# hzheng40/irbfn

Measured on AMD Instinct MI355X. Metric: RBF-net evals/s (B queries x N centres), forward, higher is better.
Workload: dtype f32 (distances and Phi x W on f16 MFMA: exact fixed-point heads + float tails, hi/lo operand pairs; f32 accumulate)

## Files before the change

irbfn_amd/csrc/pack_all.hip:

```cpp
#include <hip/hip_runtime.h>
#include <math.h>
#include <stdint.h>

#include "rbf_forward_gram.h"

namespace irbfn {

constexpr int kPackBlock = 256;
constexpr int kStatsCentres = 1024;
constexpr int kStatsVals = 18;
constexpr int kGramLdsMax = gram_chunk_bytes(8);

struct PackArgs {
  const float* __restrict__ centers;
  const float* __restrict__ log_sigs;
  const float* __restrict__ kernel;
  const float* __restrict__ bias;
  float* __restrict__ rec;
  float* __restrict__ bias_out;
  float* __restrict__ sig2;
  float* __restrict__ recm;
  float* __restrict__ oscale;
  unsigned char* __restrict__ f16_img;
  unsigned char* __restrict__ gram_img;
  GramHdr* __restrict__ hdr;
  float* __restrict__ part;
// ... 245 lines not shown
__device__ __forceinline__ void gram_image_body(const PackArgs& a, int c, unsigned char* simg, GramHdr& hs, float* tot) {
  const int tid = threadIdx.x;
  if (tid < kStatsVals) {
    float m = a.part[tid];
    for (int b = 1; b < a.nbS; ++b) m = fmaxf(m, a.part[(size_t)b * kStatsVals + tid]);
    tot[tid] = m;
  }
  __syncthreads();
  if (tid == 0) {
    hs = gram_header(tot, a.D, a.bclass, a.gscale);
    if (c == 0) *a.hdr = hs;
  }
  __syncthreads();
  const GramHdr h = hs;
  const int NT = a.NT, D = a.D;
  const int CB = gram_chunk_bytes(NT);
  unsigned char* p = simg;
  for (int it = tid; it < kF16Chunk * 16; it += kPackBlock) {
    const int part = it >> 5, kk = it & 31;
    const int reg = c / a.cpr, kr = (c - reg * a.cpr) * kF16Chunk + kk;
    const int n = reg * a.KR + kr;
    const bool real = kr < a.KR;
    const int ct = kk >> 4, row = kk & 15;
    _Float16* head = reinterpret_cast<_Float16*>(p + ct * 512);
    auto put_head = [&](int s, double v, int T) { head[((s >> 2) * 16 + row) * 4 + (s & 3)] = (_Float16)(float)(v * gram_pow2(T - gram_ax(T))); };
    auto put_tail = [&](int s, double v, int T) {
      const int half = s >> 5, g = (s >> 3) & 3, j = s & 7;
      _Float16* tail = reinterpret_cast<_Float16*>(p + kGramHeadBytes + (ct * 2 + half) * 1024);
      tail[(g * 16 + row) * 8 + j] = (_Float16)(float)(v * gram_pow2(T - gram_ax(T)));
    };
    double alpha = 0.0, beta = 0.0;
    if (h.ok) {
      const double s2 = real ? (double)expf(-2.0f * a.log_sigs[n]) : 1.0;
      gram_alpha_beta(a.bclass, s2, a.gscale, alpha, beta);
      if (!real) alpha = 0.0;
    }
    auto centre_value = [&](const GramSlot sl) -> double {
      if (!h.ok || sl.kind == 0) return 0.0;
      if (sl.kind == 1) {
        double nC[3] = {0.0, 0.0, 0.0};
        if (real && sl.dim < D) gram_parts_d(-2.0 * alpha * ((double)a.centers[(size_t)n * D + sl.dim] - (double)h.r[sl.dim]), h.ec, nC);
        return sl.q == 0 ? nC[0] : (sl.q == 1 ? nC[1] : nC[2]);
      }
      if (sl.kind == 2) {
// ... 6 lines not shown
        for (int i = 0; i < D && i < kGramDims; ++i) {
          const double cp = (double)a.centers[(size_t)n * D + i] - (double)h.r[i];
          c2 += alpha * cp * cp;
        }
      gram_parts_c2(c2, h.e2, n2);
      return sl.p == 0 ? n2[0] : (sl.p == 1 ? n2[1] : (sl.p == 2 ? n2[2] : n2[3]));
    };
    {
      const GramSlot sl = gram_head_slot(part);
      put_head(part, centre_value(sl), gram_T(h, sl));
    }
    for (int i = 0; i < 4; ++i) {
      const GramSlot sl = gram_tail_slot(4 * part + i);
      put_tail(4 * part + i, centre_value(sl), gram_T(h, sl));
    }
    const int g = row >> 2, j = ct * 4 + (row & 3);
    for (int wt = 0; wt < NT; ++wt) {
      _Float16* wh = reinterpret_cast<_Float16*>(p + kGramOpBytes + (size_t)wt * 2 * kF16WBytes);
      _Float16* wl = wh + kF16WBytes / 2;
      const int oo = part, o = wt * 16 + oo;
      float w = 0.0f;
      if (real && o < a.O) w = a.kernel[(size_t)(n % a.K) * a.O + o] / a.oscale[o];
      _Float16 hh, ll;
      split_static_f16(w, hh, ll);
      wh[(g * 16 + oo) * 8 + j] = hh;
      wl[(g * 16 + oo) * 8 + j] = ll;
    }
  }
  __syncthreads();
  uint4* dst = reinterpret_cast<uint4*>(a.gram_img + (size_t)c * CB);
// ... 78 lines not shown
```

irbfn_amd/csrc/rbf_forward_gram.h:

```cpp
#pragma once

#include "rbf_forward_f16_narrow.h"

namespace irbfn {

typedef _Float16 h4_t __attribute__((ext_vector_type(4)));

constexpr int kGramHeadBytes = 2 * 64 * 8;
constexpr int kGramTailBytes = 2 * 2 * 64 * 16;
constexpr int kGramOpBytes = kGramHeadBytes + kGramTailBytes;
constexpr int gram_chunk_bytes(int NT = 1) { return kGramOpBytes + NT * 2 * kF16WBytes; }
constexpr int kGramChunkBytes = gram_chunk_bytes(1);
constexpr int kGramDims = 8;
#ifndef IRBFN_GRAM_RING
#define IRBFN_GRAM_RING 5
#endif
constexpr int kGramRing = IRBFN_GRAM_RING;
#ifndef IRBFN_GRAM_WAVES
#define IRBFN_GRAM_WAVES 4
#endif

struct GramHdr {
  float r[8];
  int ex, ec, eq, ea, e2;
  int ok;
  float cabs, amax, cmax, c2max;
};
// ... 3 lines not shown
__host__ __device__ constexpr int gram_comb_q(int m) { return m == 0 ? 1 : (m == 1 ? 0 : (m == 2 ? 2 : (m == 3 ? 0 : 1))); }
__host__ __device__ constexpr GramSlot gram_head_slot(int s) {
  const int g = s >> 2, j = s & 3;
  return j < 2 ? GramSlot{1, 2 * g + j, 0, 0}
               : (j == 2 ? (g == 0 ? GramSlot{2, 0, 0, 0} : (g == 1 ? GramSlot{3, 0, 0, 0} : (g == 2 ? GramSlot{3, 0, 1, 0} : GramSlot{0, 0, 0, 0})))
                         : GramSlot{0, 0, 0, 0});
}
__host__ __device__ constexpr GramSlot gram_tail_slot(int s) {
  const int hf = s >> 5, g = (s >> 3) & 3, j = s & 7;
  const int m = hf * 3 + (j - 5);
  return j < 5 ? GramSlot{1, 2 * g + hf, gram_comb_p(j), gram_comb_q(j)}
               : (g == 0 ? (m < 5 ? GramSlot{2, 0, gram_comb_p(m), gram_comb_q(m)} : GramSlot{3, 0, 2, 0})
                         : (g == 1 && hf == 0 && j == 5 ? GramSlot{3, 0, 3, 0} : GramSlot{0, 0, 0, 0}));
}
static_assert(kGramDims == 8, "four lane groups x two coordinates");
__host__ __device__ inline int gram_T(const GramHdr& h, const GramSlot sl) {
  return sl.kind == 1 ? h.ex + h.ec - 11 * (sl.p + sl.q) : (sl.kind == 2 ? h.eq + h.ea - 11 * (sl.p + sl.q) : h.e2 - 11 * sl.p);
}
__host__ __device__ inline int gram_ax(int T) { return (T + 1) >> 1; }

template <int BC>
__host__ __device__ constexpr float gram_phi_scale() { return BC == BC_IMQ ? 128.0f : kPhiScale; }

#ifdef IRBFN_GRAM_STAMPS
__device__ unsigned long long g_gram_stamps[64];
#define IRBFN_GRAM_T() __builtin_amdgcn_s_memtime()
#define IRBFN_GRAM_PHASE(k)                                                                            \
  do {                                                                                                 \
    asm volatile("s_waitcnt vmcnt(0) lgkmcnt(0)" ::: "memory");                                        \
    if (blockIdx.x < 2 && threadIdx.x == 0) {                                                          \
// ... 75 lines not shown
                                                 float (&rv)[2]) {
#pragma unroll
  for (int c = 0; c < 2; ++c) rv[c] = hp->r[2 * g + c];
#pragma unroll
  for (int t = 0; t < 2; ++t)
#pragma unroll
    for (int c = 0; c < 2; ++c) {
      const int i = 2 * g + c;
      const bool in = i < DC && i < a.Dreal;
      const float v = a.x[qrow[t] * a.Dreal + (in ? i : 0)];
      xv[t][c] = in ? v : 0.0f;
    }
}

template <int DC>
__device__ __forceinline__ bool gram_query_operands(const F16Args& a, const GramHdr* hp, const float (&xin)[2][2], const float (&rin)[2],
                                                    int g, h4_t (&bhd)[2], h8_t (&btl)[2][2]) {
#pragma clang fp contract(off)
  static_assert(DC <= kGramDims, "eight coordinate slots");
  const int ex = hp->ex, ec = hp->ec, eq = hp->eq, ea = hp->ea, e2 = hp->e2;
  GramHdr hx;
  hx.ex = ex; hx.ec = ec; hx.eq = eq; hx.ea = ea; hx.e2 = e2;
  bool bad = hp->ok == 0;
  const float xinv = __builtin_ldexpf(1.0f, -ex), qinv = __builtin_ldexpf(1.0f, -eq);
  const float xlim = __builtin_ldexpf(1.0f, ex) * 0.999f, qlim = __builtin_ldexpf(1.0f, eq) * 0.999f;
  auto scale_of = [&](const GramSlot sl) -> float { return sl.kind == 0 ? 0.0f : __builtin_ldexpf(1.0f, gram_ax(gram_T(hx, sl))); };
  float rr[2];
#pragma unroll
  for (int c = 0; c < 2; ++c) {
    rr[c] = (2 * g + c < DC) ? -rin[c] : 0.0f;
  }
#pragma unroll
  for (int t = 0; t < 2; ++t) {
    float nx[2][3], nq[3];
    float qh = 0.0f, ql = 0.0f;
#pragma unroll
    for (int c = 0; c < 2; ++c) {
      const float xv = xin[t][c];
      const float sh = xv + rr[c];
      const float bb = sh - xv;
      const float sl = (xv - (sh - bb)) + (rr[c] - bb);
      bad = bad || !(__builtin_fabsf(sh) < xlim);
      gram_parts_f(sh, sl, xinv, nx[c]);
      const float ph = sh * sh;
      const float pl = __builtin_fmaf(sh, sh, -ph) + 2.0f * sh * sl;
      const float th = qh + ph;
      const float tb = th - qh;
      ql += ((qh - (th - tb)) + (ph - tb)) + pl;
      qh = th;
    }
#pragma unroll
    for (int off = 16; off <= 32; off *= 2) {
      const float oh = __shfl_xor(qh, off), ol = __shfl_xor(ql, off);
      const float th = qh + oh;
      const float tb = th - qh;
      ql = ((qh - (th - tb)) + (oh - tb)) + (ql + ol);
      qh = th;
    }
    bad = bad || !(qh < qlim);
    gram_parts_f(qh, ql, qinv, nq);
    {
      const float sc = scale_of(gram_head_slot(0));
      const float f2 = g == 0 ? nq[0] * scale_of(gram_head_slot(2))
                              : (g == 1 ? scale_of(gram_head_slot(4 + 2)) : (g == 2 ? scale_of(gram_head_slot(8 + 2)) : 0.0f));
      bhd[t][0] = (_Float16)(nx[0][0] * sc);
      bhd[t][1] = (_Float16)(nx[1][0] * sc);
      bhd[t][2] = (_Float16)f2;
      bhd[t][3] = (_Float16)0.0f;
    }
#pragma unroll
    for (int hf = 0; hf < 2; ++hf) {
#pragma unroll
      for (int j = 0; j < 5; ++j) {
        const GramSlot sl = gram_tail_slot(32 * hf + j);
        btl[t][hf][j] = (_Float16)(nx[hf][sl.p] * scale_of(sl));
      }
#pragma unroll
      for (int j = 5; j < 8; ++j) {
        const GramSlot s0 = gram_tail_slot(32 * hf + j), s1 = gram_tail_slot(32 * hf + 8 + j);
        const float v0 = s0.kind == 2 ? nq[s0.p] * scale_of(s0) : scale_of(s0);
        const float v1 = scale_of(s1);
        btl[t][hf][j] = (_Float16)(g == 0 ? v0 : (g == 1 ? v1 : 0.0f));
      }
    }
  }
  return bad;
}
template <int DC>
__device__ __forceinline__ bool gram_query_operands(const F16Args& a, const GramHdr* hp, const long (&qrow)[2], int g, h4_t (&bhd)[2],
                                                    h8_t (&btl)[2][2]) {
  float xv[2][2], rv[2];
  gram_query_loads<DC>(a, hp, qrow, g, xv, rv);
  return gram_query_operands<DC>(a, hp, xv, rv, g, bhd, btl);
}
static_assert(gram_head_slot(0).kind == 1 && gram_head_slot(4 * 3 + 1).dim == 7 && gram_head_slot(2).kind == 2 && gram_head_slot(6).kind == 3 &&
              gram_head_slot(10).kind == 3 && gram_head_slot(10).p == 1 && gram_head_slot(14).kind == 0 && gram_head_slot(3).kind == 0, "head slots");
static_assert(gram_tail_slot(32 + 8 * 2 + 4).kind == 1 && gram_tail_slot(32 + 8 * 2 + 4).dim == 5 && gram_tail_slot(5).kind == 2 &&
              gram_tail_slot(32 + 6).kind == 2 && gram_tail_slot(32 + 7).kind == 3 && gram_tail_slot(32 + 7).p == 2 && gram_tail_slot(8 + 5).kind == 3 &&
              gram_tail_slot(8 + 5).p == 3 && gram_tail_slot(8 + 6).kind == 0 && gram_tail_slot(16 + 5).kind == 0 && gram_tail_slot(32 + 8 + 5).kind == 0, "tail slots");

__device__ __forceinline__ void gram_heads(const h4_t (&a)[2], const h4_t (&b)[2], f4_t (&u)[2][2]) {
  asm("v_mfma_f32_16x16x16_f16 %0, %4, %6, 0\n v_mfma_f32_16x16x16_f16 %1, %5, %6, 0\n v_mfma_f32_16x16x16_f16 %2, %4, %7, 0\n "
      "v_mfma_f32_16x16x16_f16 %3, %5, %7, 0\n s_nop 4"
      : "=&v"(u[0][0]), "=&v"(u[0][1]), "=&v"(u[1][0]), "=&v"(u[1][1])
      : "v"(a[0]), "v"(a[1]), "v"(b[0]), "v"(b[1]));
}
__device__ __forceinline__ void gram_heads2(const h4_t& a, const h4_t (&b)[2], f4_t (&u)[2]) {
  asm("v_mfma_f32_16x16x16_f16 %0, %2, %3, 0\n v_mfma_f32_16x16x16_f16 %1, %2, %4, 0\n s_nop 4"
      : "=&v"(u[0]), "=&v"(u[1])
      : "v"(a), "v"(b[0]), "v"(b[1]));
}

__device__ __forceinline__ void gram_heads2c(const h4_t& a, const h4_t (&b)[2], const f4_t& c, f4_t (&u)[2]) {
  asm("v_mfma_f32_16x16x16_f16 %0, %2, %3, %5\n v_mfma_f32_16x16x16_f16 %1, %2, %4, %5\n s_nop 4"
      : "=&v"(u[0]), "=&v"(u[1])
      : "v"(a), "v"(b[0]), "v"(b[1]), "v"(c));
}

__device__ __forceinline__ void gram_distances_at(const unsigned char* l8, const unsigned char* l16, const h4_t (&bhd)[2],
                                                  const h8_t (&btl)[2][2], f4_t (&u)[2][2]) {
  h4_t ahd[2];
  h8_t atl[2][2];
#pragma unroll
  for (int ct = 0; ct < 2; ++ct) {
    ahd[ct] = *reinterpret_cast<const h4_t*>(l8 + ct * 512);
    atl[ct][0] = *reinterpret_cast<const h8_t*>(l16 + kGramHeadBytes + (ct * 2 + 0) * 1024);
    atl[ct][1] = *reinterpret_cast<const h8_t*>(l16 + kGramHeadBytes + (ct * 2 + 1) * 1024);
  }
  gram_heads(ahd, bhd, u);
#pragma unroll
  for (int hf = 0; hf < 2; ++hf)
#pragma unroll
    for (int t = 0; t < 2; ++t)
#pragma unroll
      for (int ct = 0; ct < 2; ++ct)
        u[t][ct] = __builtin_amdgcn_mfma_f32_16x16x32_f16(atl[ct][hf], btl[t][hf], u[t][ct], 0, 0, 0);
}
__device__ __forceinline__ void gram_distances(const unsigned char* buf, int lane, const h4_t (&bhd)[2], const h8_t (&btl)[2][2],
                                               f4_t (&u)[2][2]) {
  gram_distances_at(buf + lane * 8, buf + lane * 16, bhd, btl, u);
}

template <int DC, int BC, bool FINITE_R2 = false>
__device__ __forceinline__ void gram_valu_args(const F16Args& a, const long (&qrow)[2], int g, const float* recs, float (&t16)[16]) {
  constexpr int RF = f16_rf(DC);
#pragma unroll
  for (int t = 0; t < 2; ++t) {
    float xq[DC];
#pragma unroll
    for (int d = 0; d < DC; ++d) xq[d] = d < a.Dreal ? a.x[qrow[t] * a.Dreal + d] : 0.0f;
#pragma unroll
    for (int j = 0; j < 8; ++j) {
      const float* rp = recs + ((j >> 2) * 16 + 4 * g + (j & 3)) * RF;
      float r2 = 0.0f;
#pragma unroll
// ... 18 lines not shown
```

irbfn_amd/csrc/rbf_forward_gram.hip:

```cpp
#include <hip/hip_fp16.h>
#include <stdint.h>
#include <stdio.h>
#include <stdlib.h>

#include "rbf_forward_gram_body.h"

namespace irbfn {

template <int DC, int BC>
__global__ __launch_bounds__(1024, IRBFN_GRAM_WAVES) void rbf_fwd_f16gram(const GramArgs ga) {
  extern __shared__ __attribute__((aligned(16))) unsigned char lds[];
  gram_body<DC, BC, false>(ga, F16Roll{}, -1, lds);
}

template <int DC, int BC>
__global__ __launch_bounds__(1024, IRBFN_GRAM_WAVES) void rbf_tick_f16gram(const GramArgs ga, const F16Roll rl, const int mode) {
  extern __shared__ __attribute__((aligned(16))) unsigned char lds[];
  gram_body<DC, BC, true>(ga, rl, mode, lds);
}

static int gram_nt(const irbfn_net* net) { return (net->O + 15) / 16; }

bool gram_eligible(const irbfn_net* net) {
  return f16_eligible(net) && net->DC <= kGramDims;
}

size_t gram_image_bytes(const irbfn_net* net) {
  const int nchunks = (net->N + kF16Chunk - 1) / kF16Chunk;
  return (size_t)nchunks * gram_chunk_bytes(gram_nt(net));
}

size_t gram_header_bytes() { return sizeof(GramHdr); }

#ifdef IRBFN_GRAM_STAMPS
extern "C" int irbfn_debug_gram_stamps(unsigned long long* out64) {
  return (int)hipMemcpyFromSymbol(out64, HIP_SYMBOL(g_gram_stamps), sizeof(unsigned long long) * 64);
}
#endif

size_t gram_lds_bytes(int S, int QG, bool tick, bool gamma) {
  size_t ring = (size_t)S * kGramRing * kGramChunkBytes;
  if (gamma) ring += (size_t)S * QG * 128 * sizeof(float);
  else ring += (size_t)QG * 32 * sizeof(float);
  size_t red = (size_t)S * QG * 2 * 4 * 64 + (size_t)QG * 32;
// ... 31 lines not shown
```

irbfn_amd/csrc/rbf_forward_gram_body.h:

```cpp
#pragma once

#include "rbf_forward_gram.h"

namespace irbfn {

struct GramGamma {
  const float* __restrict__ gamma;
  int R, cpr;
};

template <int DC, int BC, bool ROLL, bool GAMMA = false>
__device__ __forceinline__ void gram_body(const GramArgs& ga, const F16Roll& rl, int mode, unsigned char* lds,
                                          [[maybe_unused]] const GramGamma gm = GramGamma{nullptr, 1, 1}) {
  static_assert(DC <= kGramDims, "eight coordinate slots");
  const F16Args& a = ga.f;
  constexpr int CBL = f16_chunk_bytes(DC);
  constexpr int CB = kGramChunkBytes;
  const int tid = threadIdx.x, lane = tid & 63;
  IRBFN_GRAM_PHASE(GP_ENTRY);
  const int wave = __builtin_amdgcn_readfirstlane(tid >> 6);
  const int S = a.S, QG = a.QG;
  int slice = 0;
#pragma unroll
  for (int s2 = 1; s2 < 8; ++s2) slice += wave >= s2 * QG ? 1 : 0;
  const int qg = wave - slice * QG;
  const int g = lane >> 4, n = lane & 15;
  const long q0 = ((long)blockIdx.x * QG + qg) * 32;
  const GramHdr* hp = ga.hdr;
  long qrow[2];
#pragma unroll
  for (int t = 0; t < 2; ++t) {
    long q = q0 + t * 16 + n;
// ... 9 lines not shown
      float xg[2][DC];
#pragma unroll
      for (int t = 0; t < 2; ++t)
#pragma unroll
        for (int d = 0; d < DC; ++d) xg[t][d] = a.x[qrow[t] * a.Dreal + (d < gr.nsplit ? d : 0)];
#pragma unroll
      for (int t = 0; t < 2; ++t) {
        float gv = gr.n_ranges > 0 ? 1.0f : 0.0f;
#pragma unroll
        for (int d = 0; d < DC; ++d)
          if (d < gr.nsplit && gr.n_ranges > 0) gv *= gate_factor(xg[t][d], gr.lo[d], gr.hi[d], gr.delta[d]);
        if (g == 0) gpark[t * 16 + n] = gv;
      }
    }
  }
  h4_t bhd[2];
  h8_t btl[2][2];
  const bool bad = gram_query_operands<DC>(a, hp, xop, rop, g, bhd, btl);
  const bool wave_bad = __builtin_amdgcn_readfirstlane(__builtin_amdgcn_ballot_w64(bad) != 0ull ? 1 : 0) != 0;
#ifdef IRBFN_GRAM_STAMPS
  asm volatile("" ::"s"((int)wave_bad), "v"(bhd[1]), "v"(btl[1][1]));
#endif
  IRBFN_GRAM_PHASE(GP_OPERANDS);

  const unsigned nch = (unsigned)a.nchunks;
  const int c0 = (int)(nch * (unsigned)slice / (unsigned)S), c1 = (int)(nch * (unsigned)(slice + 1) / (unsigned)S);
  const int na = c1 - c0;
  const int nsteps = ga.nsteps;
  unsigned char* ring = lds + (size_t)slice * kGramRing * CB;
  constexpr int NVI = CB / 1024;
  [[maybe_unused]] int npc = 0;
#pragma unroll
  for (int p = 0; p < NVI; ++p) npc += qg + p * QG < NVI ? 1 : 0;
  [[maybe_unused]] const unsigned char* gnext = ga.gimg + (size_t)c0 * CB + qg * 1024 + lane * 16;
  auto stage = [&](int k, int buf) __attribute__((always_inline)) {
    if (k >= na) return;
    unsigned char* dst = ring + buf * CB;
    if constexpr (GAMMA) {
      const unsigned char* gp = ga.gimg + (size_t)(c0 + k) * CB + lane * 16;
      for (int v = qg; v < NVI; v += QG)
        __builtin_amdgcn_global_load_lds((gptr_t)(gp + v * 1024), (lptr_t)(dst + v * 1024), 16, 0, 0);
    } else {
      if (npc > 0) {
        const unsigned char* gp = gnext;
        unsigned char* lp = dst + qg * 1024;
        __builtin_amdgcn_global_load_lds((gptr_t)gp, (lptr_t)lp, 16, 0, 0);
        for (int p = 1; p < npc; ++p) {
          gp += QG * 1024;
          lp += QG * 1024;
          __builtin_amdgcn_global_load_lds((gptr_t)gp, (lptr_t)lp, 16, 0, 0);
        }
      }
      gnext += CB;
    }
  };
  auto step_barrier = [&]() { asm volatile("s_waitcnt vmcnt(0) lgkmcnt(0)\n\ts_barrier" ::: "memory"); };
  auto next3 = [&](int b3) { return b3 == kGramRing - 1 ? 0 : b3 + 1; };
  constexpr int kGramPer = (kGramRing - 1) / 2;
  static_assert(kGramRing == 2 * kGramPer + 1 && kGramPer >= 1, "ring = 2 x (steps per barrier) + 1");
  [[maybe_unused]] float* gtile = nullptr;
  [[maybe_unused]] const float* grow = nullptr;
  [[maybe_unused]] int glim = 0;
  if constexpr (GAMMA) {
    static_assert(kGramPer <= 2, "a period's weights are one dword per lane");
    gtile = reinterpret_cast<float*>(lds + (size_t)S * kGramRing * CB) + wave * 128;
    const long qb = q0 < a.B ? q0 : a.B - 1;
    grow = gm.gamma + qb * (long)gm.R;
    glim = a.B - 1 - qb < 31 ? (int)(a.B - 1 - qb) : 31;
// ... 59 lines not shown
      acl[t] = __builtin_amdgcn_mfma_f32_16x16x32_f16(ah, bl, acl[t], 0, 0, 0);
    }
  };

#pragma unroll
  for (int k = 0; k <= kGramPer; ++k) stage(k, k);
  gamma_stage(0);
  step_barrier();
  IRBFN_GRAM_PHASE(GP_BARRIER1);
#pragma unroll
  for (int k = kGramPer + 1; k < kGramRing; ++k) stage(k, k);
  gamma_stage(1);
  IRBFN_GRAM_PHASE(GP_LOOP0);
  if (!wave_bad) {
    f4_t ua[2][2], ub[2][2];
    if (na > 0) gram_distances(ring, lane, bhd, btl, ua);
    asm volatile("s_nop 7\n\ts_nop 7" ::: "memory");
    [[maybe_unused]] unsigned long long tph[5] = {0, 0, 0, 0, 0};
    unsigned o8 = (unsigned)(slice * kGramRing * CB) + lane * 8, o16 = (unsigned)(slice * kGramRing * CB) + lane * 16;
    if constexpr (!GAMMA) asm volatile("" : "+v"(o8), "+v"(o16));
    const unsigned char* const r8 = lds + o8;
    const unsigned char* const r16 = lds + o16;
    static_assert((kGramRing - 1) * CB + kGramOpBytes + kF16WBytes + 16 <= 65536, "the offset field of ds_read has 16 bits");
    auto one_step = [&](int i, int b0, int par, f4_t (&ucur)[2][2], f4_t (&unxt)[2][2], bool all = false) __attribute__((always_inline)) {
      const int b1 = next3(b0);
      [[maybe_unused]] const unsigned long long t0 = IRBFN_GRAM_T();
      if (all || i + 1 < na) gram_distances_at(r8 + b1 * CB, r16 + b1 * CB, bhd, btl, unxt);
      if (all || i < na) {
        gamma_read(i);
        float t16[16];
        products(t16, r16 + b0 * CB, [&](float (&o)[16]) { trans16<BC>(ucur, o); });
      }
      [[maybe_unused]] const unsigned long long t2 = IRBFN_GRAM_T();
#ifdef IRBFN_GRAM_STAMPS
      t_refill = 0;
#endif
      end_of_step(i, b0, par);
      [[maybe_unused]] const unsigned long long t4 = IRBFN_GRAM_T();
#ifdef IRBFN_GRAM_STAMPS
      const unsigned long long t3 = t_refill != 0 ? t_refill : t4;
      tph[1] += t2 - t0; tph[2] += t3 - t2; tph[3] += t4 - t3; tph[4] += 1;
#endif
// ... 62 lines not shown
```

irbfn_amd/csrc/rbf_forward_gram_gamma.hip:

```cpp
#ifdef IRBFN_GRAM_STAMPS
#undef IRBFN_GRAM_STAMPS
#endif
#include <hip/hip_fp16.h>
#include <stdint.h>

#include "rbf_forward_gram_body.h"

namespace irbfn {

template <int DC, int BC>
__global__ __launch_bounds__(1024, IRBFN_GRAM_WAVES) void rbf_fwd_f16gram_gamma(const GramArgs ga, const GramGamma gm) {
  extern __shared__ __attribute__((aligned(16))) unsigned char lds[];
  gram_body<DC, BC, false, true>(ga, F16Roll{}, -1, lds, gm);
}

template <int DC, int BC>
__global__ __launch_bounds__(1024, IRBFN_GRAM_WAVES) void rbf_tick_f16gram_gamma(const GramArgs ga, const GramGamma gm, const F16Roll rl,
                                                                                 const int mode) {
  extern __shared__ __attribute__((aligned(16))) unsigned char lds[];
  gram_body<DC, BC, true, true>(ga, rl, mode, lds, gm);
}

int gram_gamma_cpr(const irbfn_net* net) { return (net->K + kF16Chunk - 1) / kF16Chunk; }

// ... 9 lines not shown
  if (!gram_gamma_eligible(net) || net->R == 1) return IRBFN_OK;
  if (!net->vjp_flags) {
    void* f = nullptr;
    hipError_t e = hipMalloc(&f, 64 * sizeof(int));
    if (e == hipSuccess) e = hipMemset(f, 0, 64 * sizeof(int));
    if (e != hipSuccess) {
      g_last_hip_error = (int)e;
      if (f) (void)hipFree(f);
      return IRBFN_ERR_HIP;
    }
    net->vjp_flags = static_cast<int*>(f);
  }
  if (net->gram_img) return IRBFN_OK;
  const size_t nchunks = (size_t)net->R * gram_gamma_cpr(net);
  void* bufs[5] = {nullptr, nullptr, nullptr, nullptr, nullptr};
  const size_t bytes[5] = {nchunks * f16_chunk_bytes(net->DC, 1), 128 * sizeof(float), nchunks * kGramChunkBytes, sizeof(GramHdr),
                           pack_partials_bytes(net)};
  for (int i = 0; i < 5; ++i) {
    const hipError_t e = hipMalloc(&bufs[i], bytes[i]);
    if (e != hipSuccess) {
      g_last_hip_error = (int)e;
      for (int j = 0; j < i; ++j) (void)hipFree(bufs[j]);
      return IRBFN_ERR_HIP;
    }
  }
  net->f16_img = static_cast<unsigned char*>(bufs[0]);
  net->f16_oscale = static_cast<float*>(bufs[1]);
  net->gram_img = static_cast<unsigned char*>(bufs[2]);
  net->gram_hdr = bufs[3];
  net->pack_part = static_cast<float*>(bufs[4]);
  net->gamma_packed = 0;
// ... 39 lines not shown
```

irbfn_amd/csrc/rbf_forward_gram_wide.h:

```cpp
#pragma once

#include "rbf_forward_gram.h"

namespace irbfn {

template <int DC, int BC, int NT, int MODE>
__device__ __forceinline__ void wide_gram_body(const GramArgs& ga, const F16Roll& rl, unsigned char* lds) {
  const F16Args& a = ga.f;
  constexpr int CBL = f16_chunk_bytes(DC, NT);
  constexpr int CB = gram_chunk_bytes(NT);
  constexpr int NVI = CB / 1024;
  const int tid = threadIdx.x, lane = tid & 63;
  const int wave = __builtin_amdgcn_readfirstlane(tid >> 6);
  const int SW = a.S, QG = a.QG;
  const int slice = wave / QG, qg = wave % QG;
  const int g = lane >> 4, n = lane & 15;
  const long q0 = ((long)blockIdx.x * QG + qg) * 32;
  long qrow[2];
#pragma unroll
  for (int t = 0; t < 2; ++t) {
    long q = q0 + t * 16 + n;
    q = q < a.B ? q : a.B - 1;
    qrow[t] = q < 0 ? 0 : q;
  }
  h4_t bhd[2];
  h8_t btl[2][2];
  const bool bad = gram_query_operands<DC>(a, ga.hdr, qrow, g, bhd, btl);
  const bool wave_bad = __builtin_amdgcn_ballot_w64(bad) != 0ull;

  const int nsteps = (a.nchunks + SW - 1) / SW;
  const int c0 = slice * nsteps;
  const int c1 = (c0 + nsteps) < a.nchunks ? (c0 + nsteps) : a.nchunks;
  const int na = c1 > c0 ? c1 - c0 : 0;
  unsigned char* ring = lds + (size_t)slice * 3 * CB;
  auto stage = [&](int k, int buf) {
    if (k >= na) return;
    const unsigned char* gp = ga.gimg + (size_t)(c0 + k) * CB + lane * 16;
    unsigned char* dst = ring + buf * CB;
    for (int v = qg; v < NVI; v += QG)
      __builtin_amdgcn_global_load_lds((gptr_t)(gp + v * 1024), (lptr_t)(dst + v * 1024), 16, 0, 0);
  };
  auto step_barrier = [&]() { asm volatile("s_waitcnt vmcnt(0) lgkmcnt(0)\n\ts_barrier" ::: "memory"); };
  auto next3 = [&](int b3) { return b3 == 2 ? 0 : b3 + 1; };

  f4_t acc[2][NT], acl[2][NT];
#pragma unroll
  for (int t = 0; t < 2; ++t)
#pragma unroll
    for (int ct = 0; ct < NT; ++ct) { acc[t][ct] = f4_t{0, 0, 0, 0}; acl[t][ct] = f4_t{0, 0, 0, 0}; }
  auto split16 = [&](const float (&t16)[16], h8_t (&ah)[2], h8_t (&al)[2]) {
#pragma unroll
    for (int t = 0; t < 2; ++t) {
// ... 21 lines not shown
        acc[t][ct] = __builtin_amdgcn_mfma_f32_16x16x32_f16(ah[t], bh, acc[t][ct], 0, 0, 0);
        acl[t][ct] = __builtin_amdgcn_mfma_f32_16x16x32_f16(al[t], bh, acl[t][ct], 0, 0, 0);
        acl[t][ct] = __builtin_amdgcn_mfma_f32_16x16x32_f16(ah[t], bl, acl[t][ct], 0, 0, 0);
      }
      __builtin_amdgcn_sched_barrier(0);
      bh = nbh; bl = nbl;
    }
  };

  stage(0, 0);
  stage(1, 1);
  step_barrier();
  stage(2, 2);
  if (!wave_bad) {
    f4_t u[2][2];
    if (na > 0) gram_distances(ring, lane, bhd, btl, u);
    asm volatile("s_nop 7\n\ts_nop 7" ::: "memory");
    int b0 = 0;
    for (int i = 0; i < nsteps; ++i) {
      const int b1 = next3(b0);
      if (i < na) {
        h8_t ah[2], al[2];
        {
          float t16[16];
          trans16<BC>(u, t16);
          split16(t16, ah, al);
        }
        if (i + 1 < na) gram_distances(ring + b1 * CB, lane, bhd, btl, u);
        products(ah, al, ring + b0 * CB);
      }
      step_barrier();
      stage(i + 3, b0);
      b0 = b1;
    }
  } else {
    int b0 = 0;
    for (int i = 0; i < nsteps; ++i) {
      if (i < na) {
        h8_t ah[2], al[2];
        {
          float t16[16];
          gram_valu_args<DC, BC>(a, qrow, g, reinterpret_cast<const float*>(a.img + (size_t)(c0 + i) * CBL), t16);
          trans_block<BC, 16>(t16);
// ... 14 lines not shown
```

irbfn_amd/csrc/rbf_vjp_gram.hip:

```cpp
#include <hip/hip_fp16.h>
#include <stdint.h>
#include <stdio.h>

#include "rbf_forward_gram.h"
#include "rbf_vjp_f16.h"

namespace irbfn {

constexpr int kVgDist = 2 * (512 + 2 * 1024);
constexpr int kVgGA = 1024 + 2048;
constexpr int kVgBlock = kVgDist + kVgGA + 2 * 2048;
constexpr int kVgPieces = kVgBlock / 1024;
constexpr int kVgOC = 10;
__host__ __device__ constexpr int vg_gamma_gain(int bc) { return bc == BC_GAUSS ? 14 : (bc == BC_IQ ? 0 : 7); }
__host__ __device__ constexpr int vg_exp_a(int bc, bool gamma = false) { return bc == BC_GAUSS && !gamma ? 9 : 16; }
__host__ __device__ constexpr int vg_exp_b(int bc, bool gamma = false) { return bc == BC_GAUSS && !gamma ? 10 : 17; }
constexpr float kVgCrossA = 1.0f / 32.0f, kVgCrossB = 1.0f / 64.0f;
static_assert(kVgCrossA * kVgCrossB == kLoScale, "cross terms of the (hi, lo) scheme");

__device__ __forceinline__ float vg_pow2_ceil_scale(float mx) {
  if (!(mx > 0.0f) || !(mx < 3.0e38f)) return 1.0f;
  int e;
  (void)frexpf(mx, &e);
  return ldexpf(1.0f, e);
// ... 467 lines not shown

template <int MODE>
static int launch_vjp_gram_mode(irbfn_net* net, const float* x, const float* gout, int64_t B, unsigned char* qblk, const float* bmax,
                                int nbmax, float* scales, int* flag, int gen, float* part, int QSB, int Npad, hipStream_t s,
                                const float* gtile = nullptr) {
  const long nqb = (B + 31) / 32;
  const GramHdr* hdr = reinterpret_cast<const GramHdr*>(net->gram_hdr);
  const dim3 pg((unsigned)nqb), pb(192);
  const int rc = dispatch<3, 4, 7, 8>(net->DC, [&](auto dc) {
    return launch_kernel<vjp_pack_blocks_gram_kernel<dc(), MODE>>(pg, pb, 0, s, x, gout, bmax, nbmax, net->f16_oscale, hdr, qblk, scales, flag,
                                                                 gen, net->gate(), (long)B, net->D, net->O,
                                                                 vg_exp_a(net->bclass, gtile != nullptr), gtile != nullptr ? 1 : 0);
  });
  if (rc != IRBFN_OK) return rc;
  VjpGArgs a;
  a.qblk = qblk; a.scales = scales; a.gimg = net->gram_img; a.hdr = hdr; a.flag = flag; a.gen = gen; a.rec = net->rec; a.sig2 = net->sig2;
  a.oscale = net->f16_oscale; a.part = part;
  a.nqb = nqb; a.O = net->O; a.OP = net->OP; a.N = net->N; a.S = net->S; a.Npad = Npad;
  a.bpb = (int)((nqb + QSB - 1) / QSB);
  a.cstride = gram_chunk_bytes((net->O + 15) / 16);
  a.nchunks = (net->N + 31) / 32;
  a.gscale = gauss_scale(net->basis);
  if (gtile != nullptr) {
    if constexpr (MODE == VG_ALL) {
      const VjpGGamma gm = {gtile, net->R, net->K, gram_gamma_cpr(net)};
      a.nchunks = gm.R * gm.cpr;
      const dim3 gg((a.nchunks + 3) / 4, QSB);
      const size_t lds = (size_t)3 * vg_slot_bytes(VG_ALL);
      return dispatch<3, 4, 7, 8>(net->DC, [&](auto dc) {
        return dispatch<BC_GAUSS, BC_IQ, BC_IMQ>(net->bclass, [&](auto bc) {
          return a.O <= kVgOC ? launch_kernel<rbf_vjp_f16gram_gamma<dc(), bc(), true>>(gg, dim3(256), lds, s, a, gm)
                              : launch_kernel<rbf_vjp_f16gram_gamma<dc(), bc(), false>>(gg, dim3(256), lds, s, a, gm);
        });
      });
    }
// ... 61 lines not shown
```

Before: 948.8 million.

## Fold Gram distance head and tail operands into two 16x16x32 MFMA slots

Repacks the per-chunk centre operands so the distance Gram product uses two 16x16x32 f16 MFMA k-slices instead of one 16x16x16 head MFMA plus two tail MFMAs per tile. Query operands are built from shared parts, with a cross-lane shuffle supplying coordinates owned by other lane groups. The forward kernels read a smaller operand block per chunk, which means fewer LDS reads and fewer MFMA issues per step. The old head/tail layout is kept after the forward region so the VJP path keeps working, at the cost of a larger global image and a wider chunk stride.

```diff
diff --git a/irbfn_amd/csrc/pack_all.hip b/irbfn_amd/csrc/pack_all.hip
--- a/irbfn_amd/csrc/pack_all.hip
+++ b/irbfn_amd/csrc/pack_all.hip
@@ -9,7 +9,7 @@
 constexpr int kPackBlock = 256;
 constexpr int kStatsCentres = 1024;
 constexpr int kStatsVals = 18;
-constexpr int kGramLdsMax = gram_chunk_bytes(8);
+constexpr int kGramLdsMax = gram_chunk_stride(8);
 
 struct PackArgs {
   const float* __restrict__ centers;
@@ -285,7 +285,8 @@
   __syncthreads();
   const GramHdr h = hs;
   const int NT = a.NT, D = a.D;
-  const int CB = gram_chunk_bytes(NT);
+  const int CB = gram_chunk_stride(NT);
+  unsigned char* const pv = simg + gram_chunk_bytes(NT);
   unsigned char* p = simg;
   for (int it = tid; it < kF16Chunk * 16; it += kPackBlock) {
     const int part = it >> 5, kk = it & 31;
@@ -293,12 +294,16 @@
     const int n = reg * a.KR + kr;
     const bool real = kr < a.KR;
     const int ct = kk >> 4, row = kk & 15;
-    _Float16* head = reinterpret_cast<_Float16*>(p + ct * 512);
+    _Float16* head = reinterpret_cast<_Float16*>(pv + ct * 512);
     auto put_head = [&](int s, double v, int T) { head[((s >> 2) * 16 + row) * 4 + (s & 3)] = (_Float16)(float)(v * gram_pow2(T - gram_ax(T))); };
     auto put_tail = [&](int s, double v, int T) {
       const int half = s >> 5, g = (s >> 3) & 3, j = s & 7;
-      _Float16* tail = reinterpret_cast<_Float16*>(p + kGramHeadBytes + (ct * 2 + half) * 1024);
+      _Float16* tail = reinterpret_cast<_Float16*>(pv + kGramHeadBytes + (ct * 2 + half) * 1024);
       tail[(g * 16 + row) * 8 + j] = (_Float16)(float)(v * gram_pow2(T - gram_ax(T)));
+    };
+    auto put_fold = [&](int o, int k, double v, int T) {
+      _Float16* op = reinterpret_cast<_Float16*>(p + (ct * 2 + o) * 1024);
+      op[((k >> 3) * 16 + row) * 8 + (k & 7)] = (_Float16)(float)(v * gram_pow2(T - gram_ax(T)));
     };
     double alpha = 0.0, beta = 0.0;
     if (h.ok) {
@@ -335,6 +340,11 @@
       const GramSlot sl = gram_tail_slot(4 * part + i);
       put_tail(4 * part + i, centre_value(sl), gram_T(h, sl));
     }
+    for (int i = 0; i < 4; ++i) {
+      const int o = part >> 3, k = 4 * (part & 7) + i;
+      const GramSlot sl = gram_fold_slot(o, k);
+      put_fold(o, k, centre_value(sl), gram_T(h, sl));
+    }
     const int g = row >> 2, j = ct * 4 + (row & 3);
     for (int wt = 0; wt < NT; ++wt) {
       _Float16* wh = reinterpret_cast<_Float16*>(p + kGramOpBytes + (size_t)wt * 2 * kF16WBytes);
diff --git a/irbfn_amd/csrc/rbf_forward_gram.h b/irbfn_amd/csrc/rbf_forward_gram.h
--- a/irbfn_amd/csrc/rbf_forward_gram.h
+++ b/irbfn_amd/csrc/rbf_forward_gram.h
@@ -6,11 +6,13 @@
 
 typedef _Float16 h4_t __attribute__((ext_vector_type(4)));
 
+constexpr int kGramOpBytes = 2 * 2 * 64 * 16;
+constexpr int gram_chunk_bytes(int NT = 1) { return kGramOpBytes + NT * 2 * kF16WBytes; }
+constexpr int kGramChunkBytes = gram_chunk_bytes(1);
 constexpr int kGramHeadBytes = 2 * 64 * 8;
 constexpr int kGramTailBytes = 2 * 2 * 64 * 16;
-constexpr int kGramOpBytes = kGramHeadBytes + kGramTailBytes;
-constexpr int gram_chunk_bytes(int NT = 1) { return kGramOpBytes + NT * 2 * kF16WBytes; }
-constexpr int kGramChunkBytes = gram_chunk_bytes(1);
+constexpr int kGramVjpBytes = kGramHeadBytes + kGramTailBytes;
+constexpr int gram_chunk_stride(int NT = 1) { return gram_chunk_bytes(NT) + kGramVjpBytes; }
 constexpr int kGramDims = 8;
 #ifndef IRBFN_GRAM_RING
 #define IRBFN_GRAM_RING 5
@@ -44,6 +46,52 @@
                          : (g == 1 && hf == 0 && j == 5 ? GramSlot{3, 0, 3, 0} : GramSlot{0, 0, 0, 0}));
 }
 static_assert(kGramDims == 8, "four lane groups x two coordinates");
+
+__host__ __device__ constexpr GramSlot gram_fold_slot(int o, int k) {
+  const int g = k >> 3, j = k & 7;
+  if (o == 0 && g < 2)
+    return j < 2 ? GramSlot{1, 2 * g + j, 0, 0}
+                 : (j < 4 ? GramSlot{1, 4 + 2 * g + (j - 2), 0, 0}
+                          : (g == 0 ? (j == 4 ? GramSlot{2, 0, 0, 0} : GramSlot{0, 0, 0, 0})
+                                    : (j == 4 ? GramSlot{3, 0, 0, 0} : (j == 5 ? GramSlot{3, 0, 1, 0} : GramSlot{0, 0, 0, 0}))));
+  if (o == 0)
+    return j < 5 ? GramSlot{1, 2 * g, gram_comb_p(j), gram_comb_q(j)}
+                 : (j < 7 ? GramSlot{1, 2 * (g - 2) + (j - 5), 1, 1} : (g == 2 ? GramSlot{3, 0, 3, 0} : GramSlot{0, 0, 0, 0}));
+  if (g < 2) return GramSlot{1, 2 * g + (j >> 2), gram_comb_p(j & 3), gram_comb_q(j & 3)};
+  if (j < 5) return GramSlot{1, 2 * g + 1, gram_comb_p(j), gram_comb_q(j)};
+  const int m = (g - 2) * 3 + (j - 5);
+  return m < 5 ? GramSlot{2, 0, gram_comb_p(m), gram_comb_q(m)} : GramSlot{3, 0, 2, 0};
+}
+__host__ __device__ constexpr bool gram_slot_is_head(const GramSlot sl) { return sl.kind == 3 ? sl.p < 2 : (sl.kind != 0 && sl.p + sl.q == 0); }
+__host__ __device__ constexpr int gram_fold_count(int kind, int dim, int p, int q) {
+  int c = 0;
+  for (int o = 0; o < 2; ++o)
+    for (int k = 0; k < 32; ++k) {
+      const GramSlot sl = gram_fold_slot(o, k);
+      c += (sl.kind == kind && sl.dim == dim && sl.p == p && sl.q == q) ? 1 : 0;
+    }
+  return c;
+}
+__host__ __device__ constexpr bool gram_fold_tables_ok() {
+  int used = 0;
+  for (int o = 0; o < 2; ++o)
+    for (int k = 0; k < 32; ++k) {
+      const GramSlot sl = gram_fold_slot(o, k);
+      used += sl.kind != 0 ? 1 : 0;
+      if (sl.kind != 0 && gram_slot_is_head(sl) != (o == 0 && k < 16)) return false;
+    }
+  if (used != 8 * 6 + 6 + 4) return false;
+  for (int p = 0; p < 3; ++p)
+    for (int q = 0; p + q < 3; ++q) {
+      for (int d = 0; d < kGramDims; ++d)
+        if (gram_fold_count(1, d, p, q) != 1) return false;
+      if (gram_fold_count(2, 0, p, q) != 1) return false;
+    }
+  for (int p = 0; p < 4; ++p)
+    if (gram_fold_count(3, 0, p, 0) != 1) return false;
+  return true;
+}
+static_assert(gram_fold_tables_ok(), "folded slot tables");
 __host__ __device__ inline int gram_T(const GramHdr& h, const GramSlot sl) {
   return sl.kind == 1 ? h.ex + h.ec - 11 * (sl.p + sl.q) : (sl.kind == 2 ? h.eq + h.ea - 11 * (sl.p + sl.q) : h.e2 - 11 * sl.p);
 }
@@ -149,17 +197,14 @@
 }
 
 template <int DC>
-__device__ __forceinline__ bool gram_query_operands(const F16Args& a, const GramHdr* hp, const float (&xin)[2][2], const float (&rin)[2],
-                                                    int g, h4_t (&bhd)[2], h8_t (&btl)[2][2]) {
+__device__ __forceinline__ bool gram_query_parts(const GramHdr* hp, const float (&xin)[2][2], const float (&rin)[2], int g,
+                                                 float (&nx)[2][2][3], float (&nq)[2][3]) {
 #pragma clang fp contract(off)
   static_assert(DC <= kGramDims, "eight coordinate slots");
-  const int ex = hp->ex, ec = hp->ec, eq = hp->eq, ea = hp->ea, e2 = hp->e2;
-  GramHdr hx;
-  hx.ex = ex; hx.ec = ec; hx.eq = eq; hx.ea = ea; hx.e2 = e2;
+  const int ex = hp->ex, eq = hp->eq;
   bool bad = hp->ok == 0;
   const float xinv = __builtin_ldexpf(1.0f, -ex), qinv = __builtin_ldexpf(1.0f, -eq);
   const float xlim = __builtin_ldexpf(1.0f, ex) * 0.999f, qlim = __builtin_ldexpf(1.0f, eq) * 0.999f;
-  auto scale_of = [&](const GramSlot sl) -> float { return sl.kind == 0 ? 0.0f : __builtin_ldexpf(1.0f, gram_ax(gram_T(hx, sl))); };
   float rr[2];
 #pragma unroll
   for (int c = 0; c < 2; ++c) {
@@ -167,7 +212,6 @@
   }
 #pragma unroll
   for (int t = 0; t < 2; ++t) {
-    float nx[2][3], nq[3];
     float qh = 0.0f, ql = 0.0f;
 #pragma unroll
     for (int c = 0; c < 2; ++c) {
@@ -176,7 +220,7 @@
       const float bb = sh - xv;
       const float sl = (xv - (sh - bb)) + (rr[c] - bb);
       bad = bad || !(__builtin_fabsf(sh) < xlim);
-      gram_parts_f(sh, sl, xinv, nx[c]);
+      gram_parts_f(sh, sl, xinv, nx[t][c]);
       const float ph = sh * sh;
       const float pl = __builtin_fmaf(sh, sh, -ph) + 2.0f * sh * sl;
       const float th = qh + ph;
@@ -193,7 +237,23 @@
       qh = th;
     }
     bad = bad || !(qh < qlim);
-    gram_parts_f(qh, ql, qinv, nq);
+    gram_parts_f(qh, ql, qinv, nq[t]);
+  }
+  return bad;
+}
+
+template <int DC>
+__device__ __forceinline__ bool gram_query_operands(const F16Args& a, const GramHdr* hp, const float (&xin)[2][2], const float (&rin)[2],
+                                                    int g, h4_t (&bhd)[2], h8_t (&btl)[2][2]) {
+  GramHdr hx;
+  hx.ex = hp->ex; hx.ec = hp->ec; hx.eq = hp->eq; hx.ea = hp->ea; hx.e2 = hp->e2;
+  auto scale_of = [&](const GramSlot sl) -> float { return sl.kind == 0 ? 0.0f : __builtin_ldexpf(1.0f, gram_ax(gram_T(hx, sl))); };
+  float nxa[2][2][3], nqa[2][3];
+  const bool bad = gram_query_parts<DC>(hp, xin, rin, g, nxa, nqa);
+#pragma unroll
+  for (int t = 0; t < 2; ++t) {
+    const float (&nx)[2][3] = nxa[t];
+    const float (&nq)[3] = nqa[t];
     {
       const float sc = scale_of(gram_head_slot(0));
       const float f2 = g == 0 ? nq[0] * scale_of(gram_head_slot(2))
@@ -221,6 +281,47 @@
   }
   return bad;
 }
+
+template <int DC>
+__device__ __forceinline__ bool gram_query_operands_fold(const F16Args& a, const GramHdr* hp, const float (&xin)[2][2],
+                                                         const float (&rin)[2], int g, h8_t (&bq)[2][2]) {
+  typedef _Float16 h2_t __attribute__((ext_vector_type(2)));
+  GramHdr hx;
+  hx.ex = hp->ex; hx.ec = hp->ec; hx.eq = hp->eq; hx.ea = hp->ea; hx.e2 = hp->e2;
+  auto scale_of = [&](const GramSlot sl) -> float { return sl.kind == 0 ? 0.0f : __builtin_ldexpf(1.0f, gram_ax(gram_T(hx, sl))); };
+  float nxa[2][2][3], nqa[2][3];
+  const bool bad = gram_query_parts<DC>(hp, xin, rin, g, nxa, nqa);
+  const bool lower = g < 2;
+#pragma unroll
+  for (int t = 0; t < 2; ++t) {
+    const float (&nx)[2][3] = nxa[t];
+    const float (&nq)[3] = nqa[t];
+    const float sc0 = scale_of(GramSlot{1, 0, 0, 0}), sc11 = scale_of(GramSlot{1, 0, 1, 1});
+    const h2_t mine = lower ? h2_t{(_Float16)(nx[0][1] * sc11), (_Float16)(nx[1][1] * sc11)}
+                            : h2_t{(_Float16)(nx[0][0] * sc0), (_Float16)(nx[1][0] * sc0)};
+    const h2_t theirs = __builtin_bit_cast(h2_t, __shfl_xor(__builtin_bit_cast(int, mine), 32));
+    auto value = [&](const GramSlot sl, int gg) -> float {
+      if (sl.kind == 0) return 0.0f;
+      if (sl.kind == 2) return nq[sl.p] * scale_of(sl);
+      if (sl.kind == 3) return scale_of(sl);
+      return nx[sl.dim & 1][sl.p] * scale_of(sl);
+    };
+#pragma unroll
+    for (int o = 0; o < 2; ++o)
+#pragma unroll
+      for (int j = 0; j < 8; ++j) {
+        _Float16 v[4];
+#pragma unroll
+        for (int gg = 0; gg < 4; ++gg) {
+          const GramSlot sl = gram_fold_slot(o, 8 * gg + j);
+          const bool foreign = sl.kind == 1 && (sl.dim >> 1) != gg;
+          v[gg] = foreign ? theirs[sl.dim & 1] : (_Float16)value(sl, gg);
+        }
+        bq[t][o][j] = g == 0 ? v[0] : (g == 1 ? v[1] : (g == 2 ? v[2] : v[3]));
+      }
+  }
+  return bad;
+}
 template <int DC>
 __device__ __forceinline__ bool gram_query_operands(const F16Args& a, const GramHdr* hp, const long (&qrow)[2], int g, h4_t (&bhd)[2],
                                                     h8_t (&btl)[2][2]) {
@@ -228,18 +329,18 @@
   gram_query_loads<DC>(a, hp, qrow, g, xv, rv);
   return gram_query_operands<DC>(a, hp, xv, rv, g, bhd, btl);
 }
+template <int DC>
+__device__ __forceinline__ bool gram_query_operands_fold(const F16Args& a, const GramHdr* hp, const long (&qrow)[2], int g, h8_t (&bq)[2][2]) {
+  float xv[2][2], rv[2];
+  gram_query_loads<DC>(a, hp, qrow, g, xv, rv);
+  return gram_query_operands_fold<DC>(a, hp, xv, rv, g, bq);
+}
 static_assert(gram_head_slot(0).kind == 1 && gram_head_slot(4 * 3 + 1).dim == 7 && gram_head_slot(2).kind == 2 && gram_head_slot(6).kind == 3 &&
               gram_head_slot(10).kind == 3 && gram_head_slot(10).p == 1 && gram_head_slot(14).kind == 0 && gram_head_slot(3).kind == 0, "head slots");
 static_assert(gram_tail_slot(32 + 8 * 2 + 4).kind == 1 && gram_tail_slot(32 + 8 * 2 + 4).dim == 5 && gram_tail_slot(5).kind == 2 &&
               gram_tail_slot(32 + 6).kind == 2 && gram_tail_slot(32 + 7).kind == 3 && gram_tail_slot(32 + 7).p == 2 && gram_tail_slot(8 + 5).kind == 3 &&
               gram_tail_slot(8 + 5).p == 3 && gram_tail_slot(8 + 6).kind == 0 && gram_tail_slot(16 + 5).kind == 0 && gram_tail_slot(32 + 8 + 5).kind == 0, "tail slots");
 
-__device__ __forceinline__ void gram_heads(const h4_t (&a)[2], const h4_t (&b)[2], f4_t (&u)[2][2]) {
-  asm("v_mfma_f32_16x16x16_f16 %0, %4, %6, 0\n v_mfma_f32_16x16x16_f16 %1, %5, %6, 0\n v_mfma_f32_16x16x16_f16 %2, %4, %7, 0\n "
-      "v_mfma_f32_16x16x16_f16 %3, %5, %7, 0\n s_nop 4"
-      : "=&v"(u[0][0]), "=&v"(u[0][1]), "=&v"(u[1][0]), "=&v"(u[1][1])
-      : "v"(a[0]), "v"(a[1]), "v"(b[0]), "v"(b[1]));
-}
 __device__ __forceinline__ void gram_heads2(const h4_t& a, const h4_t (&b)[2], f4_t (&u)[2]) {
   asm("v_mfma_f32_16x16x16_f16 %0, %2, %3, 0\n v_mfma_f32_16x16x16_f16 %1, %2, %4, 0\n s_nop 4"
       : "=&v"(u[0]), "=&v"(u[1])
@@ -252,28 +353,24 @@
       : "v"(a), "v"(b[0]), "v"(b[1]), "v"(c));
 }
 
-__device__ __forceinline__ void gram_distances_at(const unsigned char* l8, const unsigned char* l16, const h4_t (&bhd)[2],
-                                                  const h8_t (&btl)[2][2], f4_t (&u)[2][2]) {
-  h4_t ahd[2];
-  h8_t atl[2][2];
-#pragma unroll
-  for (int ct = 0; ct < 2; ++ct) {
-    ahd[ct] = *reinterpret_cast<const h4_t*>(l8 + ct * 512);
-    atl[ct][0] = *reinterpret_cast<const h8_t*>(l16 + kGramHeadBytes + (ct * 2 + 0) * 1024);
-    atl[ct][1] = *reinterpret_cast<const h8_t*>(l16 + kGramHeadBytes + (ct * 2 + 1) * 1024);
-  }
-  gram_heads(ahd, bhd, u);
-#pragma unroll
-  for (int hf = 0; hf < 2; ++hf)
-#pragma unroll
-    for (int t = 0; t < 2; ++t)
-#pragma unroll
-      for (int ct = 0; ct < 2; ++ct)
-        u[t][ct] = __builtin_amdgcn_mfma_f32_16x16x32_f16(atl[ct][hf], btl[t][hf], u[t][ct], 0, 0, 0);
-}
-__device__ __forceinline__ void gram_distances(const unsigned char* buf, int lane, const h4_t (&bhd)[2], const h8_t (&btl)[2][2],
-                                               f4_t (&u)[2][2]) {
-  gram_distances_at(buf + lane * 8, buf + lane * 16, bhd, btl, u);
+__device__ __forceinline__ void gram_distances_at(const unsigned char* l16, const h8_t (&bq)[2][2], f4_t (&u)[2][2]) {
+  h8_t aq[2][2];
+#pragma unroll
+  for (int ct = 0; ct < 2; ++ct)
+#pragma unroll
+    for (int o = 0; o < 2; ++o) aq[ct][o] = *reinterpret_cast<const h8_t*>(l16 + (ct * 2 + o) * 1024);
+  const f4_t z = {0.0f, 0.0f, 0.0f, 0.0f};
+#pragma unroll
+  for (int t = 0; t < 2; ++t)
+#pragma unroll
+    for (int ct = 0; ct < 2; ++ct) u[t][ct] = __builtin_amdgcn_mfma_f32_16x16x32_f16(aq[ct][0], bq[t][0], z, 0, 0, 0);
+#pragma unroll
+  for (int t = 0; t < 2; ++t)
+#pragma unroll
+    for (int ct = 0; ct < 2; ++ct) u[t][ct] = __builtin_amdgcn_mfma_f32_16x16x32_f16(aq[ct][1], bq[t][1], u[t][ct], 0, 0, 0);
+}
+__device__ __forceinline__ void gram_distances(const unsigned char* buf, int lane, const h8_t (&bq)[2][2], f4_t (&u)[2][2]) {
+  gram_distances_at(buf + lane * 16, bq, u);
 }
 
 template <int DC, int BC, bool FINITE_R2 = false>
diff --git a/irbfn_amd/csrc/rbf_forward_gram.hip b/irbfn_amd/csrc/rbf_forward_gram.hip
--- a/irbfn_amd/csrc/rbf_forward_gram.hip
+++ b/irbfn_amd/csrc/rbf_forward_gram.hip
@@ -27,7 +27,7 @@
 
 size_t gram_image_bytes(const irbfn_net* net) {
   const int nchunks = (net->N + kF16Chunk - 1) / kF16Chunk;
-  return (size_t)nchunks * gram_chunk_bytes(gram_nt(net));
+  return (size_t)nchunks * gram_chunk_stride(gram_nt(net));
 }
 
 size_t gram_header_bytes() { return sizeof(GramHdr); }
diff --git a/irbfn_amd/csrc/rbf_forward_gram_body.h b/irbfn_amd/csrc/rbf_forward_gram_body.h
--- a/irbfn_amd/csrc/rbf_forward_gram_body.h
+++ b/irbfn_amd/csrc/rbf_forward_gram_body.h
@@ -16,6 +16,7 @@
   const F16Args& a = ga.f;
   constexpr int CBL = f16_chunk_bytes(DC);
   constexpr int CB = kGramChunkBytes;
+  constexpr int CST = gram_chunk_stride(1);
   const int tid = threadIdx.x, lane = tid & 63;
   IRBFN_GRAM_PHASE(GP_ENTRY);
   const int wave = __builtin_amdgcn_readfirstlane(tid >> 6);
@@ -55,12 +56,11 @@
       }
     }
   }
-  h4_t bhd[2];
-  h8_t btl[2][2];
-  const bool bad = gram_query_operands<DC>(a, hp, xop, rop, g, bhd, btl);
+  h8_t bq[2][2];
+  const bool bad = gram_query_operands_fold<DC>(a, hp, xop, rop, g, bq);
   const bool wave_bad = __builtin_amdgcn_readfirstlane(__builtin_amdgcn_ballot_w64(bad) != 0ull ? 1 : 0) != 0;
 #ifdef IRBFN_GRAM_STAMPS
-  asm volatile("" ::"s"((int)wave_bad), "v"(bhd[1]), "v"(btl[1][1]));
+  asm volatile("" ::"s"((int)wave_bad), "v"(bq[1][0]), "v"(bq[1][1]));
 #endif
   IRBFN_GRAM_PHASE(GP_OPERANDS);
 
@@ -73,12 +73,12 @@
   [[maybe_unused]] int npc = 0;
 #pragma unroll
   for (int p = 0; p < NVI; ++p) npc += qg + p * QG < NVI ? 1 : 0;
-  [[maybe_unused]] const unsigned char* gnext = ga.gimg + (size_t)c0 * CB + qg * 1024 + lane * 16;
+  [[maybe_unused]] const unsigned char* gnext = ga.gimg + (size_t)c0 * CST + qg * 1024 + lane * 16;
   auto stage = [&](int k, int buf) __attribute__((always_inline)) {
     if (k >= na) return;
     unsigned char* dst = ring + buf * CB;
     if constexpr (GAMMA) {
-      const unsigned char* gp = ga.gimg + (size_t)(c0 + k) * CB + lane * 16;
+      const unsigned char* gp = ga.gimg + (size_t)(c0 + k) * CST + lane * 16;
       for (int v = qg; v < NVI; v += QG)
         __builtin_amdgcn_global_load_lds((gptr_t)(gp + v * 1024), (lptr_t)(dst + v * 1024), 16, 0, 0);
     } else {
@@ -92,7 +92,7 @@
           __builtin_amdgcn_global_load_lds((gptr_t)gp, (lptr_t)lp, 16, 0, 0);
         }
       }
-      gnext += CB;
+      gnext += CST;
     }
   };
   auto step_barrier = [&]() { asm volatile("s_waitcnt vmcnt(0) lgkmcnt(0)\n\ts_barrier" ::: "memory"); };
@@ -182,18 +182,17 @@
   IRBFN_GRAM_PHASE(GP_LOOP0);
   if (!wave_bad) {
     f4_t ua[2][2], ub[2][2];
-    if (na > 0) gram_distances(ring, lane, bhd, btl, ua);
+    if (na > 0) gram_distances(ring, lane, bq, ua);
     asm volatile("s_nop 7\n\ts_nop 7" ::: "memory");
     [[maybe_unused]] unsigned long long tph[5] = {0, 0, 0, 0, 0};
-    unsigned o8 = (unsigned)(slice * kGramRing * CB) + lane * 8, o16 = (unsigned)(slice * kGramRing * CB) + lane * 16;
-    if constexpr (!GAMMA) asm volatile("" : "+v"(o8), "+v"(o16));
-    const unsigned char* const r8 = lds + o8;
+    unsigned o16 = (unsigned)(slice * kGramRing * CB) + lane * 16;
+    if constexpr (!GAMMA) asm volatile("" : "+v"(o16));
     const unsigned char* const r16 = lds + o16;
     static_assert((kGramRing - 1) * CB + kGramOpBytes + kF16WBytes + 16 <= 65536, "the offset field of ds_read has 16 bits");
     auto one_step = [&](int i, int b0, int par, f4_t (&ucur)[2][2], f4_t (&unxt)[2][2], bool all = false) __attribute__((always_inline)) {
       const int b1 = next3(b0);
       [[maybe_unused]] const unsigned long long t0 = IRBFN_GRAM_T();
-      if (all || i + 1 < na) gram_distances_at(r8 + b1 * CB, r16 + b1 * CB, bhd, btl, unxt);
+      if (all || i + 1 < na) gram_distances_at(r16 + b1 * CB, bq, unxt);
       if (all || i < na) {
         gamma_read(i);
         float t16[16];
diff --git a/irbfn_amd/csrc/rbf_forward_gram_gamma.hip b/irbfn_amd/csrc/rbf_forward_gram_gamma.hip
--- a/irbfn_amd/csrc/rbf_forward_gram_gamma.hip
+++ b/irbfn_amd/csrc/rbf_forward_gram_gamma.hip
@@ -47,7 +47,7 @@
   if (net->gram_img) return IRBFN_OK;
   const size_t nchunks = (size_t)net->R * gram_gamma_cpr(net);
   void* bufs[5] = {nullptr, nullptr, nullptr, nullptr, nullptr};
-  const size_t bytes[5] = {nchunks * f16_chunk_bytes(net->DC, 1), 128 * sizeof(float), nchunks * kGramChunkBytes, sizeof(GramHdr),
+  const size_t bytes[5] = {nchunks * f16_chunk_bytes(net->DC, 1), 128 * sizeof(float), nchunks * gram_chunk_stride(1), sizeof(GramHdr),
                            pack_partials_bytes(net)};
   for (int i = 0; i < 5; ++i) {
     const hipError_t e = hipMalloc(&bufs[i], bytes[i]);
diff --git a/irbfn_amd/csrc/rbf_forward_gram_wide.h b/irbfn_amd/csrc/rbf_forward_gram_wide.h
--- a/irbfn_amd/csrc/rbf_forward_gram_wide.h
+++ b/irbfn_amd/csrc/rbf_forward_gram_wide.h
@@ -9,6 +9,7 @@
   const F16Args& a = ga.f;
   constexpr int CBL = f16_chunk_bytes(DC, NT);
   constexpr int CB = gram_chunk_bytes(NT);
+  constexpr int CST = gram_chunk_stride(NT);
   constexpr int NVI = CB / 1024;
   const int tid = threadIdx.x, lane = tid & 63;
   const int wave = __builtin_amdgcn_readfirstlane(tid >> 6);
@@ -23,9 +24,8 @@
     q = q < a.B ? q : a.B - 1;
     qrow[t] = q < 0 ? 0 : q;
   }
-  h4_t bhd[2];
-  h8_t btl[2][2];
-  const bool bad = gram_query_operands<DC>(a, ga.hdr, qrow, g, bhd, btl);
+  h8_t bq[2][2];
+  const bool bad = gram_query_operands_fold<DC>(a, ga.hdr, qrow, g, bq);
   const bool wave_bad = __builtin_amdgcn_ballot_w64(bad) != 0ull;
 
   const int nsteps = (a.nchunks + SW - 1) / SW;
@@ -35,7 +35,7 @@
   unsigned char* ring = lds + (size_t)slice * 3 * CB;
   auto stage = [&](int k, int buf) {
     if (k >= na) return;
-    const unsigned char* gp = ga.gimg + (size_t)(c0 + k) * CB + lane * 16;
+    const unsigned char* gp = ga.gimg + (size_t)(c0 + k) * CST + lane * 16;
     unsigned char* dst = ring + buf * CB;
     for (int v = qg; v < NVI; v += QG)
       __builtin_amdgcn_global_load_lds((gptr_t)(gp + v * 1024), (lptr_t)(dst + v * 1024), 16, 0, 0);
@@ -87,7 +87,7 @@
   stage(2, 2);
   if (!wave_bad) {
     f4_t u[2][2];
-    if (na > 0) gram_distances(ring, lane, bhd, btl, u);
+    if (na > 0) gram_distances(ring, lane, bq, u);
     asm volatile("s_nop 7\n\ts_nop 7" ::: "memory");
     int b0 = 0;
     for (int i = 0; i < nsteps; ++i) {
@@ -99,7 +99,7 @@
           trans16<BC>(u, t16);
           split16(t16, ah, al);
         }
-        if (i + 1 < na) gram_distances(ring + b1 * CB, lane, bhd, btl, u);
+        if (i + 1 < na) gram_distances(ring + b1 * CB, lane, bq, u);
         products(ah, al, ring + b0 * CB);
       }
       step_barrier();
diff --git a/irbfn_amd/csrc/rbf_vjp_gram.hip b/irbfn_amd/csrc/rbf_vjp_gram.hip
--- a/irbfn_amd/csrc/rbf_vjp_gram.hip
+++ b/irbfn_amd/csrc/rbf_vjp_gram.hip
@@ -505,11 +505,15 @@
   });
   if (rc != IRBFN_OK) return rc;
   VjpGArgs a;
-  a.qblk = qblk; a.scales = scales; a.gimg = net->gram_img; a.hdr = hdr; a.flag = flag; a.gen = gen; a.rec = net->rec; a.sig2 = net->sig2;
+  a.qblk = qblk; a.scales = scales; a.hdr = hdr; a.flag = flag; a.gen = gen; a.rec = net->rec; a.sig2 = net->sig2;
   a.oscale = net->f16_oscale; a.part = part;
   a.nqb = nqb; a.O = net->O; a.OP = net->OP; a.N = net->N; a.S = net->S; a.Npad = Npad;
   a.bpb = (int)((nqb + QSB - 1) / QSB);
-  a.cstride = gram_chunk_bytes((net->O + 15) / 16);
+  {
+    const int nt = (net->O + 15) / 16;
+    a.gimg = net->gram_img + gram_chunk_bytes(nt);
+    a.cstride = gram_chunk_stride(nt);
+  }
   a.nchunks = (net->N + 31) / 32;
   a.gscale = gauss_scale(net->basis);
   if (gtile != nullptr) {
```

Measured after the change: 1.013 billion (median of 6 runs). 1.07x the previous value.
